# tkkiran/Robust-Conditional-GAN

Measured on AMD Instinct MI355X. Metric: images/sec G+D train step (CIFAR-10 RCGAN bs=64), higher is better.
Workload: dtype bf16

## Files before the change

include/rcgan_hip.h:

```cpp
#ifndef RCGAN_HIP_H
#define RCGAN_HIP_H

#include <stddef.h>
#include <stdint.h>

#ifdef __cplusplus
extern "C" {
#endif

#define RCGAN_OK 0
#define RCGAN_EINVALID_ARG (-1)
#define RCGAN_EUNSUPPORTED_SHAPE (-2)
#define RCGAN_EWORKSPACE_TOO_SMALL (-3)
#define RCGAN_EHIP (-4)
#define RCGAN_ERCCL (-5)

#define RCGAN_F32 0
#define RCGAN_BF16 1
#define RCGAN_F16 2

#define RCGAN_ACT_NONE 0
#define RCGAN_ACT_RELU 1
#define RCGAN_ACT_LRELU 2
#define RCGAN_ACT_TANH 3
// ... 225 lines not shown
int rcgan_conv_rf_prepare(rcgan_ctx* ctx, int n, const rcgan_conv_desc* descs, const void* const* prepared, void* const* frags);
int rcgan_fragments_prepare(rcgan_ctx* ctx, const void* const* trunk_prepared, void* trunk_frag, int n, const rcgan_conv_desc* descs,
                            const void* const* prepared, void* const* frags);
int rcgan_conv2d_rf(rcgan_ctx* ctx, const rcgan_conv_desc* d, int backward, const void* x, const void* frag, const float* bias,
                    const void* mask_x, const void* residual, void* y);

int rcgan_dblock2_ok(const rcgan_conv_desc* d, const void* conv1_frag, const void* dblock2_frag);
size_t rcgan_dblock2_fragment_bytes(void);
int rcgan_fragments_prepare_dblock2(rcgan_ctx* ctx, const void* const* trunk_prepared, void* trunk_frag, int n, const rcgan_conv_desc* descs,
                                    const void* const* prepared, void* const* frags, const void* conv2_prepared,
                                    const void* shortcut_prepared, void* dblock2_frag);
int rcgan_dblock2_fwd(rcgan_ctx* ctx, const rcgan_conv_desc* d, const void* x, const void* conv1_frag, const void* dblock2_frag,
                      const float* bias1, const float* bias2, const float* bias_shortcut, void* h, void* xp, void* y);
int rcgan_dblock2_bwd(rcgan_ctx* ctx, const rcgan_conv_desc* d, const void* dy, const void* h, const void* x, const void* conv1_frag,
                      const void* dblock2_frag, void* dh, void* dx);

int rcgan_dblock1_ok(const rcgan_conv_desc* d, const void* dblock1_frag);
size_t rcgan_dblock1_fragment_bytes(void);
int rcgan_fragments_prepare_dblocks(rcgan_ctx* ctx, const void* const* trunk_prepared, void* trunk_frag, int n, const rcgan_conv_desc* descs,
                                    const void* const* prepared, void* const* frags, const void* conv2_prepared,
                                    const void* shortcut_prepared, void* dblock2_frag, const void* block1_conv2_prepared, void* dblock1_frag);
int rcgan_dblock1_fwd(rcgan_ctx* ctx, const rcgan_conv_desc* d, const void* x, const void* conv1_prepared, const void* shortcut_prepared,
                      const void* dblock1_frag, const float* bias1, const float* bias2, const float* bias_shortcut, void* h, void* xp, void* y);
size_t rcgan_proj_head_workspace_bytes(int n, int d, int v);
typedef struct {
  int n, d, v, e_dim;
  int rows_a, kind_a, kind_b;
  float weight;
  const int32_t* labels_a; const float* wts_a; float* dwts_a;
  const int32_t* labels_b; const float* wts_b; float* dwts_b;
  const void* x; void* dx;
  int x_dtype, hw, act;
  const float* E_pre;
  void* defer_ws;
  size_t defer_ws_bytes;
} rcgan_head_desc;
int rcgan_proj_head_fwd_bwd(rcgan_ctx* ctx, const rcgan_head_desc* hd, const float* feat, const float* w_out, const float* sigma_out,
                            const float* b_out, const float* table, const float* w_e, const float* sigma_e, const float* b_e,
                            float* loss_acc, float* logits, float* dfeat, float* dw_out, float* db_out, float* dtable, float* dw_e,
                            float* db_e, void* ws, size_t ws_bytes);
int rcgan_head_flush(rcgan_ctx* ctx);

typedef struct {
  float weight;
  const float* anchor_a; const float* anchor_b;
  const float* gate;
// ... 136 lines not shown
```

robust-conditional-gan_amd/_lib.py:

```python
import ctypes as C
import os

_HERE = os.path.dirname(os.path.abspath(__file__))
LIB_PATH = os.environ.get("RCGAN_LIB_PATH") or os.path.join(_HERE, "librcgan_hip.so")
LIB_PATH_F16 = os.environ.get("RCGAN_LIB_PATH_F16") or os.path.join(_HERE, "librcgan_hip_f16.so")

F32, BF16, F16 = 0, 1, 2
ACT_NONE, ACT_RELU, ACT_LRELU, ACT_TANH, ACT_SIGMOID = 0, 1, 2, 3, 4
CONV_IN_UPSAMPLE2X, CONV_IN_RELU, CONV_ACCUMULATE, CONV_FORCE_DIRECT, CONV_OUT_MEANPOOL2, CONV_RESID_UPSAMPLE2X = 1, 2, 4, 8, 16, 32
LOSS_HINGE_REAL, LOSS_HINGE_FAKE, LOSS_NEG_MEAN, LOSS_CE_ONES, LOSS_CE_ZEROS = 0, 1, 2, 3, 4
QUERY_TR_READ = 0
AUG_COLOR, AUG_TRANSLATION, AUG_CUTOUT = 1, 2, 4
AUG_POLICIES = {"color": AUG_COLOR, "translation": AUG_TRANSLATION, "cutout": AUG_CUTOUT}
F32_PRECISION_HIGHEST, F32_PRECISION_HIGH = 0, 1
F32_PRECISIONS = {"highest": F32_PRECISION_HIGHEST, "high": F32_PRECISION_HIGH}

RCGAN_EHIP, RCGAN_ERCCL = -4, -5
EINVALID_ARG, EUNSUPPORTED_SHAPE, EWORKSPACE_TOO_SMALL = -1, -2, -3
ERRORS = {-1: "RCGAN_EINVALID_ARG", -2: "RCGAN_EUNSUPPORTED_SHAPE", -3: "RCGAN_EWORKSPACE_TOO_SMALL",
          -4: "RCGAN_EHIP", -5: "RCGAN_ERCCL"}


def source_hash():
    import glob
# ... 172 lines not shown
    "rcgan_proj_logit_fwd": (I, [P, I, I, P, P, P, P]),
    "rcgan_proj_logit_bwd": (I, [P, I, I, P, P, P, P, P, P, I]),
    "rcgan_proj_logit_all_fwd": (I, [P, I, I, I, P, P, P, P]),
    "rcgan_proj_logit_all_bwd": (I, [P, I, I, I, P, P, P, P, P, P, I]),
    "rcgan_loss_fwd_bwd": (I, [P, I, I, I, P, P, F, P, P, P]),
    "rcgan_bce_onehot_fwd_bwd": (I, [P, I, I, P, P, F, P, P]),
    "rcgan_dtrunk": (I, [P, I, I, P, P, P, P, P]),
    "rcgan_dtrunk_pooled": (I, [P, I, I, P, P, P, P, P, P, P, P]),
    "rcgan_dtrunk_prepare": (I, [P, P, P]),
    "rcgan_conv_rf_ok": (I, [C.POINTER(ConvDesc)]),
    "rcgan_conv_rf_fragment_bytes": (SZ, [C.POINTER(ConvDesc)]),
    "rcgan_conv_rf_prepare": (I, [P, I, C.POINTER(ConvDesc), P, P]),
    "rcgan_fragments_prepare": (I, [P, P, P, I, C.POINTER(ConvDesc), P, P]),
    "rcgan_conv2d_rf": (I, [P, C.POINTER(ConvDesc), I, P, P, P, P, P, P]),
    "rcgan_dblock2_ok": (I, [C.POINTER(ConvDesc), P, P]),
    "rcgan_dblock2_fragment_bytes": (SZ, []),
    "rcgan_fragments_prepare_dblock2": (I, [P, P, P, I, C.POINTER(ConvDesc), P, P, P, P, P]),
    "rcgan_dblock2_fwd": (I, [P, C.POINTER(ConvDesc), P, P, P, P, P, P, P, P, P]),
    "rcgan_dblock2_bwd": (I, [P, C.POINTER(ConvDesc), P, P, P, P, P, P, P]),
    "rcgan_dblock1_ok": (I, [C.POINTER(ConvDesc), P]),
    "rcgan_dblock1_fragment_bytes": (SZ, []),
    "rcgan_fragments_prepare_dblocks": (I, [P, P, P, I, C.POINTER(ConvDesc), P, P, P, P, P, P, P]),
    "rcgan_dblock1_fwd": (I, [P, C.POINTER(ConvDesc), P, P, P, P, P, P, P, P, P, P]),
    "rcgan_dtrunk_fragment_bytes": (SZ, []),
    "rcgan_head_flush": (I, [P]),
    "rcgan_proj_head_fwd_bwd": (I, [P, C.POINTER(HeadDesc)] + [P] * 16 + [P, SZ]),
    "rcgan_recover_mse_fwd_bwd": (I, [P, I, I, I, I, P, P, P, P, P, P, P, SZ]),
    "rcgan_softmax_rows_fwd": (I, [P, I, I, P, P]),
    "rcgan_softmax_rows_bwd": (I, [P, I, I, P, P, P, I]),
    "rcgan_softmax_xent_workspace_bytes": (SZ, [I]),
    "rcgan_softmax_xent_fwd_bwd": (I, [P, I, I, P, P, F, P, P, P, P, SZ]),
    "rcgan_softmax_xent_forward_fwd_bwd": (I, [P, I, I, P, P, P, F, P, P, P, P, P, P, SZ]),
    "rcgan_shortcut_a_fwd": (I, [P, I, I, I, I, I, P, P]),
    "rcgan_shortcut_a_bwd": (I, [P, I, I, I, I, I, P, P, I]),
    "rcgan_diffaugment_fwd": (I, [P, I, I, I, I, I, P, P, P, P]),
    "rcgan_diffaugment_bwd": (I, [P, I, I, I, I, I, P, P, P, I]),
    "rcgan_diffaugment_gated_fwd": (I, [P, I, I, I, I, I, P, P, P, P, P, P, P]),
    "rcgan_diffaugment_sampled_bwd": (I, [P, I, I, I, I, P, P, P, P, I]),
    "rcgan_ada_update": (I, [P, I, P, I, P, P, F, F, I]),
    "rcgan_loss_reg_fwd_bwd": (I, [P, I, I, I, P, P, F, P, P, P, C.POINTER(LossReg)]),
    "rcgan_proj_head_reg_fwd_bwd": (I, [P, C.POINTER(HeadDesc)] + [P] * 16 + [P, SZ, C.POINTER(LossReg)]),
    "rcgan_lecam_update": (I, [P, I, I, P, I, P, P, P, P, P, F]),
    "rcgan_pair_diversity_workspace_bytes": (SZ, [I]),
    "rcgan_pair_diversity_fwd_bwd": (I, [P, I, I, I, I, P, P, P, F, F, P, P, I, P, P, SZ]),
    "rcgan_class_moments_bytes": (SZ, [I, I]),
    "rcgan_class_moments_accum": (I, [P, I, I, I, P, P, P]),
# ... 72 lines not shown
```

robust-conditional-gan_amd/csrc/api.hip:

```cpp
#include "conv_wgrad.h"
#include "small_gemm.h"
#include "step_inputs.h"
#include "conv_image.h"
#include "gather_plan.h"


size_t direct_wgrad_ws_bytes(const rcgan_conv_desc* d);
template <typename T> int direct_fwd(rcgan_ctx*, const rcgan_conv_desc*, const T*, const float*, const float*, const float*, T*, int n_cols = 0);
template <typename T> int direct_dgrad(rcgan_ctx*, const rcgan_conv_desc*, const T*, const float*, const float*, const float*, const T*, T*, int);
template <typename T> int direct_wgrad(rcgan_ctx*, const rcgan_conv_desc*, const T*, const T*, float*, float*, int, void*, size_t);
template <typename T> int direct_wgrad_cols(rcgan_ctx*, const rcgan_conv_desc*, const T*, const T*, int, const float*, float*, int, void*, size_t);
size_t direct_wgrad_cols_ws_bytes(const rcgan_conv_desc* d, int c1);
template <typename T> int colsum_launch(rcgan_ctx*, const T*, long, int, float*, int, float*);
template <typename T> int linear_fwd(rcgan_ctx*, long, long, long, const T*, const float*, const float*, const float*, T*);
template <typename T> int linear_dgrad(rcgan_ctx*, long, long, long, const T*, const float*, const float*, T*, int);
template <typename T> int linear_wgrad(rcgan_ctx*, long, long, long, const T*, const T*, float*, float*, int, void*, size_t);
size_t linear_wgrad_ws_bytes(long m, long k, long n);
template <typename T> int sumpool2_masked_launch(rcgan_ctx*, int, int, int, int, const T*, const T*, T*, int);
int small_fwd_kind(const rcgan_conv_desc* d);
int small_dgrad_kind(const rcgan_conv_desc* d);
int small_wgrad_kind(const rcgan_conv_desc* d);
size_t small_wgrad_ws_bytes(const rcgan_conv_desc* d);
template <typename T> int small_fwd(rcgan_ctx*, const rcgan_conv_desc*, int, const T*, const float*, const float*, T*);
template <typename T> int small_dgrad(rcgan_ctx*, const rcgan_conv_desc*, int, const T*, const float*, T*, int);
// ... 732 lines not shown
    const bool scratch = up && a.phase == MFMA_FORM_PLAIN;
    if (scratch) a.out = (bf16_t*)target;
    a.mask = (relu && !scratch) ? (const bf16_t*)x : nullptr;
    a.resid = (const bf16_t*)residual;
    rc = mfma_conv_launch(ctx, a);
    if (rc || !scratch) return rc;
  } else if (mask == nullptr && !up && img_side(d)) {
    rc = img_dgrad(ctx, d, dy, prepared, target, acc_now);
    if (rc) return rc;
  } else if (int kind = (mask == nullptr && !up) ? small_dgrad_kind(d) : 0) {
    RC_DISPATCH_DTYPE(ctx, d->dtype, rc = small_dgrad<T>(ctx, d, kind, (const T*)dy, (const float*)prepared, (T*)target, acc_now));
    if (rc) return rc;
  } else {
    RC_DISPATCH_DTYPE(ctx, d->dtype, rc = direct_dgrad<T>(ctx, d, (const T*)dy, (const float*)prepared, nullptr, nullptr, (const T*)mask, (T*)target, acc_now));
    if (rc) return rc;
  }
  if (up) {
    RC_DISPATCH_DTYPE(ctx, d->dtype, rc = sumpool2_masked_launch<T>(ctx, d->n, d->h, d->w, d->cin, (const T*)ws, relu ? (const T*)x : (const T*)nullptr, (T*)dx, acc));
    if (rc) return rc;
  }
  return RCGAN_OK;
}

int rcgan_deconv2d_fwd(rcgan_ctx* ctx, const rcgan_conv_desc* d, const void* x, const float* w, const float* bias, void* y) {
  int rc = check_desc(ctx, d);
  if (rc) return rc;
  RC_DISPATCH_DTYPE(ctx, d->dtype, return direct_dgrad<T>(ctx, d, (const T*)x, w, nullptr, bias, (const T*)nullptr, (T*)y, 0));
  return RCGAN_OK;
}

int rcgan_deconv2d_bwd_data(rcgan_ctx* ctx, const rcgan_conv_desc* d, const void* dy, const float* w, void* dx) {
  return rcgan_deconv2d_bwd_data_cols(ctx, d, dy, w, dx, 0);
}

int rcgan_deconv2d_bwd_data_cols(rcgan_ctx* ctx, const rcgan_conv_desc* d, const void* dy, const float* w, void* dx, int n_cols) {
  int rc = check_desc(ctx, d);
  if (rc) return rc;
  RC_REQUIRE(ctx, n_cols >= 0 && n_cols <= d->cout, "n_cols %d of %d input channels", n_cols, d->cout);
  RC_DISPATCH_DTYPE(ctx, d->dtype, return direct_fwd<T>(ctx, d, (const T*)dy, w, nullptr, nullptr, (T*)dx, n_cols));
  return RCGAN_OK;
}

int rcgan_deconv2d_bwd_weight(rcgan_ctx* ctx, const rcgan_conv_desc* d, const void* x, const void* dy, float* dw, float* dbias,
                              int accumulate, void* ws, size_t ws_bytes) {
  int rc = check_desc(ctx, d);
  if (rc) return rc;
// ... 134 lines not shown
```

robust-conditional-gan_amd/csrc/conv_mfma.h:

```cpp
#pragma once
#include "common.h"

struct ImgWArgs;

struct MfmaConvArgs {
  const bf16_t* in;
  const bf16_t* wt;
  const float* bias;
  const bf16_t* mask;
  const bf16_t* resid;
  int resid_up;
  bf16_t* out;
  const bf16_t* zero;
  int N, H, W, Cin, Cout, KH, KW, PT, PL;
  int up, relu_in, accumulate;
  int cm;
  int lw, lh;
  long M;
  unsigned long long* stamps;
  const bf16_t* wph;
  int phase;
  float* stats;
  const float* bn_mean = nullptr;
  const float* bn_rstd = nullptr;
// ... 33 lines not shown
int direct_prepare_launch(rcgan_ctx* ctx, const float* w, const float* sigma, float* out, long total);
int mfma_selftest(rcgan_ctx* ctx, int* host_result);
extern int g_use_tr;
int ensure_selftest(rcgan_ctx* ctx);
int check_desc(rcgan_ctx* ctx, const rcgan_conv_desc* d);
int img_side(const rcgan_conv_desc* d);
size_t img_extra_offset(const rcgan_conv_desc* d);
size_t img_extra_bytes(const rcgan_conv_desc* d);
size_t img_wgrad_ws_bytes(const rcgan_conv_desc* d);
int img_prepare_launch(rcgan_ctx* ctx, const rcgan_conv_desc* d, const float* w, const float* sigma, void* prepared);
int img_fwd(rcgan_ctx* ctx, const rcgan_conv_desc* d, const void* x, const void* prepared, const float* bias, void* y);
int img_dgrad(rcgan_ctx* ctx, const rcgan_conv_desc* d, const void* dy, const void* prepared, void* dx, int accumulate);
bool img_fwd_bn_ok(const rcgan_conv_desc* d);
int img_fwd_bn(rcgan_ctx* ctx, const rcgan_conv_desc* d, const void* x, const void* prepared, const float* bias, void* y,
               const float* mean, const float* rstd, const float* gamma, const float* beta, const int32_t* labels, int segments, int act);
int img_wgrad_plan(rcgan_ctx* ctx, const rcgan_conv_desc* d, const void* x, const void* dy, int target_wgs, ImgWArgs* a, int* cb, int* nwg);
int img_wgrad(rcgan_ctx* ctx, const rcgan_conv_desc* d, const void* x, const void* dy, float* dw, float* dbias, int accumulate,
              void* ws, size_t ws_bytes);
int mfma_conv8_launch(rcgan_ctx* ctx, const MfmaConvArgs& a, bool wide, bool halo_patch);
bool mfma_conv8_halo_takes(const MfmaConvArgs& a);
int mfma_conv8_halo_launch(rcgan_ctx* ctx, const MfmaConvArgs& a);
bool mfma_conv8n_halo_takes(const MfmaConvArgs& a);
int mfma_conv8n_halo_launch(rcgan_ctx* ctx, const MfmaConvArgs& a);
int mfma_conv_bn_route(const MfmaConvArgs& a);
struct SmallGemmArgs;
struct StepInputsArgs;
int conv_prepare_batch_launch(rcgan_ctx* ctx, const rcgan_prepare_item* items, int n, const SmallGemmArgs* gemm = nullptr,
                              const StepInputsArgs* inputs = nullptr, const rcgan_frag_item* frags = nullptr, int n_frags = 0);
```

robust-conditional-gan_amd/csrc/conv_mfma.hip:

```cpp
#include <vector>
#include "conv_mfma.h"
#include "small_gemm.h"
#include "step_inputs.h"
#include "mfma_util.h"

#define LDS_PITCH 72

template <int BM, int BN>
__global__ __launch_bounds__(256) void conv_mfma_kernel(MfmaConvArgs a) {
  extern __shared__ __attribute__((aligned(16))) unsigned char smem[];
  bf16_t* As = (bf16_t*)smem;
  bf16_t* Bs = As + 2 * BM * LDS_PITCH;
  constexpr int AR = BM / 32, BR = BN / 32;
  constexpr int TM = BM / 2, TN = BN / 2;
  constexpr int NI = TN / 16, NJ = TM / 16;

  const int tid = threadIdx.x, lane = tid & 63, wave = tid >> 6;
  const int wm = wave & 1, wn = wave >> 1;
  const long m0 = (long)blockIdx.x * BM;
  const int co0 = blockIdx.y * BN;
  const int chunk = tid & 7, lrow = tid >> 3;
  const int K = a.KH * a.KW * a.Cin;
  const int KT = K / 64;
  const int Hs = a.up ? (a.H >> 1) : a.H, Ws = a.up ? (a.W >> 1) : a.W;
// ... 963 lines not shown
  const bool off32 = (long)a.N * a.H * a.W * a.Cin < (1L << 32);
  const long b8 = (long)cdiv(a.M, 256) * (a.Cout / 256), b8n = (long)cdiv(a.M, 256) * (a.Cout / 128);
  const bool fit8 = 4 * b8 >= 3 * (long)cdiv(b8, 256) * 256;
  if (a.Cout % 256 == 0 && a.zero != nullptr && off32 && b8 >= p8_min && fit8) return (halo && !a.stats && mfma_conv8_halo_takes(b)) ? CR_H8 : CR_P8;
  if (a.Cout % 128 == 0 && a.zero != nullptr && b8n >= p8n_min) return (halo_n && mfma_conv8n_halo_takes(b)) ? CR_H8N : CR_P8N;
  if (a.Cout % 256 == 0 && b8 >= t256_min && a.zero != nullptr) return CR_T256;
  if (a.Cout % 128 == 0 && b8n >= t256_min && a.zero != nullptr) return CR_T256N;
  if (a.Cout % 128 == 0 && (long)cdiv(a.M, 128) * (a.Cout / 128) >= t128_min) return CR_T128;
  return CR_64;
}

bool mfma_conv_is_p8(const MfmaConvArgs& a) {
  if (a.phase != MFMA_FORM_PLAIN || a.Cin % 64 || a.Cout % 64) return false;
  const ConvRoute r = mfma_conv_route(a);
  return r == CR_H8 || r == CR_P8;
}

int mfma_conv_bn_route(const MfmaConvArgs& a) {
  if (a.phase != MFMA_FORM_PLAIN || a.Cin % 64 || a.Cout % 64 || a.zero == nullptr || a.stats || a.relu_in || a.Cin > 1024) return 0;
  const ConvRoute r = mfma_conv_route(a);
  return r == CR_H8 ? 1 : r == CR_H8N ? 2 : 0;
}

int mfma_conv_launch(rcgan_ctx* ctx, const MfmaConvArgs& a_in) {
  MfmaConvArgs a = a_in;
  a.stamps = (unsigned long long*)ctx->dbg_stamps;
  if (a.Cin % 64 || a.Cout % 64) RC_FAIL(ctx, RCGAN_EUNSUPPORTED_SHAPE, "channels %d -> %d", a.Cin, a.Cout);
  const ConvRoute r = mfma_conv_route(a);
  if (a.bn_mean && !(a.phase == MFMA_FORM_PLAIN && !a.stats && !a.relu_in && a.Cin <= 1024 && a.zero != nullptr && (r == CR_H8 || r == CR_H8N)))
    RC_FAIL(ctx, RCGAN_EUNSUPPORTED_SHAPE, "batch norm on the staged input needs a halo-patch kernel (rcgan_conv_bn_in_ok)");
  if (a.stats && !(a.phase == MFMA_FORM_PLAIN && a.zero != nullptr && (r == CR_H8 || r == CR_P8)))
    RC_FAIL(ctx, RCGAN_EUNSUPPORTED_SHAPE, "tile statistics need the 256 x 256 kernel (rcgan_conv_stats_ok)");
  switch (r) {
    case CR_H8: case CR_P8: return mfma_conv8_launch(ctx, a, true, r == CR_H8);
    case CR_H8N: case CR_P8N: return mfma_conv8_launch(ctx, a, false, r == CR_H8N);
    case CR_PHASE_KS2: return a.phase == MFMA_FORM_PHASE ? launch_conv_glds_phase<64, 64, 2, 2, 1>(ctx, a) : launch_conv_glds_phase<64, 64, 2, 2, 2>(ctx, a);
    case CR_PHASE: return a.phase == MFMA_FORM_PHASE ? launch_conv_glds_phase<64, 64, 2, 1, 1>(ctx, a) : launch_conv_glds_phase<64, 64, 2, 1, 2>(ctx, a);
    case CR_T256: return launch_conv_glds<256, 256, 2>(ctx, a);
    case CR_T256N: return launch_conv_glds<256, 128, 2>(ctx, a);
    case CR_T128: return launch_conv_mfma<128, 128>(ctx, a);
    default: return launch_conv_mfma<64, 64>(ctx, a);
  }
}

int mfma_prepare_launch(rcgan_ctx* ctx, const float* w, const float* sigma, bf16_t* wt, bf16_t* wd, int T, int Cin, int Cout) {
  long total = (long)T * Cin * Cout;
// ... 58 lines not shown
```

robust-conditional-gan_amd/csrc/conv_mfma8h.hip:

```cpp
#include "conv_mfma.h"
#include "mfma_util.h"

#ifndef H8_ABLATE
#define H8_ABLATE 0
#endif

namespace {

template <int N> __device__ __forceinline__ void wait_vm() {
  if constexpr (N == 0) asm volatile("s_waitcnt vmcnt(0)" ::: "memory");
  else if constexpr (N == 1) asm volatile("s_waitcnt vmcnt(1)" ::: "memory");
  else if constexpr (N == 2) asm volatile("s_waitcnt vmcnt(2)" ::: "memory");
  else if constexpr (N == 3) asm volatile("s_waitcnt vmcnt(3)" ::: "memory");
  else if constexpr (N == 4) asm volatile("s_waitcnt vmcnt(4)" ::: "memory");
  else if constexpr (N == 5) asm volatile("s_waitcnt vmcnt(5)" ::: "memory");
  else if constexpr (N == 6) asm volatile("s_waitcnt vmcnt(6)" ::: "memory");
  else if constexpr (N == 7) asm volatile("s_waitcnt vmcnt(7)" ::: "memory");
  else if constexpr (N == 8) asm volatile("s_waitcnt vmcnt(8)" ::: "memory");
  else if constexpr (N == 9) asm volatile("s_waitcnt vmcnt(9)" ::: "memory");
  else if constexpr (N == 10) asm volatile("s_waitcnt vmcnt(10)" ::: "memory");
  else if constexpr (N == 11) asm volatile("s_waitcnt vmcnt(11)" ::: "memory");
  else if constexpr (N == 12) asm volatile("s_waitcnt vmcnt(12)" ::: "memory");
  else static_assert(N == 0, "unsupported vmcnt immediate");
}
// ... 690 lines not shown
  if (a.phase == 1) return a.up && a.wph != nullptr && (a.lw == 5 || a.lw == 6) && a.lh >= 1 && ((a.H >> 1) << (a.lw - 1)) % 256 == 0 && (a.M >> 2) % 256 == 0;
  return false;
}

template <int LW, bool RELU, bool PHM, bool BNIN = false, int NPASS = 1, bool GATHER = false>
static int launch8hn(rcgan_ctx* ctx, const MfmaConvArgs& a) {
  static bool attr_set = false;
  const size_t lds = h8n_lds_bytes(LW) + (BNIN ? 2 * H8_BN_MAX_CIN * sizeof(float) : 0);
  if (!attr_set) {
    RC_HIP(ctx, hipFuncSetAttribute((const void*)conv_mfma_h8n_kernel<LW, RELU, PHM, BNIN, NPASS, GATHER>, hipFuncAttributeMaxDynamicSharedMemorySize, (int)lds));
    attr_set = true;
  }
  dim3 grid(cdiv(a.M, 256 * NPASS), a.Cout / 128);
  {
    ProfScope ps(ctx, RCGAN_PROF_CONV_P8N, 2.0 * (double)a.M * (GATHER ? 36 : 9) * a.Cin * a.Cout,
                 2.0 * (double)a.M * (GATHER ? 16 : PHM ? 4 : 9) * a.Cin * a.Cout);
    if (BNIN && ps.on) ctx->prof_bn_in++;
    hipLaunchKernelGGL((conv_mfma_h8n_kernel<LW, RELU, PHM, BNIN, NPASS, GATHER>), grid, dim3(512), lds, ctx->stream, a);
  }
  RC_LAUNCH_CHECK(ctx);
  return RCGAN_OK;
}

int mfma_conv8n_halo_launch(rcgan_ctx* ctx, const MfmaConvArgs& a) {
  if (a.bn_mean) {
    if (a.relu_in || a.Cin > H8_BN_MAX_CIN || (a.bn_act != RCGAN_ACT_NONE && a.bn_act != RCGAN_ACT_RELU))
      RC_FAIL(ctx, RCGAN_EUNSUPPORTED_SHAPE, "batch norm on the staged patch: no input ReLU, Cin <= %d, activation none / ReLU", H8_BN_MAX_CIN);
    if (a.phase == 1) return a.lw == 6 ? launch8hn<5, false, true, true>(ctx, a) : launch8hn<4, false, true, true>(ctx, a);
    return a.lw == 5 ? launch8hn<5, false, false, true>(ctx, a) : launch8hn<4, false, false, true>(ctx, a);
  }
  if (a.phase == 2) {
    if (a.lw == 6) return a.relu_in ? launch8hn<5, true, false, false, 1, true>(ctx, a) : launch8hn<5, false, false, false, 1, true>(ctx, a);
    return a.relu_in ? launch8hn<4, true, false, false, 1, true>(ctx, a) : launch8hn<4, false, false, false, 1, true>(ctx, a);
  }
  if (a.phase == 1) {
    static int two = -1;
    if (two < 0) { const char* e = getenv("RCGAN_H8N_TWO_PASS"); two = e ? atoi(e) : 1; }
    if (two && a.Cin <= 128 && (a.M / 512) * (a.Cout / 128) >= 190) {
      if (a.lw == 6) return a.relu_in ? launch8hn<5, true, true, false, 2>(ctx, a) : launch8hn<5, false, true, false, 2>(ctx, a);
      return a.relu_in ? launch8hn<4, true, true, false, 2>(ctx, a) : launch8hn<4, false, true, false, 2>(ctx, a);
    }
    if (a.lw == 6) return a.relu_in ? launch8hn<5, true, true>(ctx, a) : launch8hn<5, false, true>(ctx, a);
    return a.relu_in ? launch8hn<4, true, true>(ctx, a) : launch8hn<4, false, true>(ctx, a);
  }
  if (a.lw == 5) return a.relu_in ? launch8hn<5, true, false>(ctx, a) : launch8hn<5, false, false>(ctx, a);
  return a.relu_in ? launch8hn<4, true, false>(ctx, a) : launch8hn<4, false, false>(ctx, a);
}
```

robust-conditional-gan_amd/csrc/conv_rf.hip:

```cpp
#include <type_traits>

#include "conv_mfma.h"
#include "mfma_util.h"
#include "rf_asm.h"

namespace {

struct RfArgs {
  const bf16_t* in;
  const bf16_t* wfrag;
  const float* bias;
  const bf16_t* mask;
  const bf16_t* resid;
  bf16_t* out;
  const bf16_t* zero;
  int accumulate, relu_in;
  int H, W, lbpi, Cout;
  int res_lw, res_lh;
  long M;
  unsigned long long* stamps;
};

constexpr int RF_ROWS = 8;
constexpr int RF_UPFRONT = 4;
// ... 238 lines not shown
                                    const void* const* prepared, void* const* frags, const void* conv2_prepared,
                                    const void* shortcut_prepared, void* dblock2_frag, const void* block1_conv2_prepared, void* dblock1_frag) {
  if (!ctx) return RCGAN_EINVALID_ARG;
  RC_REQUIRE(ctx, (block1_conv2_prepared != nullptr) == (dblock1_frag != nullptr), "the input block's copy needs its prepared filter and a destination");
  RC_REQUIRE(ctx, n >= 0 && n <= 12 && (n == 0 || (descs && prepared && frags)) && (!trunk_prepared || trunk_frag), "bad arguments");
  RC_REQUIRE(ctx, (conv2_prepared != nullptr) == (dblock2_frag != nullptr) && (shortcut_prepared != nullptr) == (dblock2_frag != nullptr),
             "the down block's copies need both prepared filters and a destination");
  RC_REQUIRE(ctx, (dblock2_frag ? DB2_FRAG_ITEMS : 0) + (dblock1_frag ? DB1_FRAG_ITEMS : 0) + (trunk_prepared ? 16 : 0) + 2 * n <=
                      (int)(sizeof(FragBatch::it) / sizeof(FragItem)),
             "more fragment items than one launch holds");
  FragBatch b;
  int m = 0, maxchunks = 0;
  if (dblock2_frag) {
    const rcgan_conv_desc d2 = {1, 16, 16, 128, 128, 3, 3, 1, RCGAN_H16, RCGAN_CONV_OUT_MEANPOOL2};
    const rcgan_conv_desc ds = {1, 8, 8, 128, 128, 1, 1, 1, RCGAN_H16, 0};
    dblock2_frag_items((const bf16_t*)conv2_prepared + mfma_prepared_sum_fwd(&d2), (const bf16_t*)shortcut_prepared,
                       (const bf16_t*)conv2_prepared + mfma_prepared_sum_bwd(&d2), (const bf16_t*)shortcut_prepared + mfma_prepared_rot(&ds),
                       (bf16_t*)dblock2_frag, b.it);
    m = DB2_FRAG_ITEMS;
    maxchunks = b.it[0].chunks;
  }
  if (dblock1_frag) {
    const rcgan_conv_desc d2 = {1, 32, 32, 128, 128, 3, 3, 1, RCGAN_H16, RCGAN_CONV_OUT_MEANPOOL2};
    dblock1_frag_items((const bf16_t*)block1_conv2_prepared + mfma_prepared_sum_fwd(&d2), (bf16_t*)dblock1_frag, b.it + m);
    if (b.it[m].chunks > maxchunks) maxchunks = b.it[m].chunks;
    m += DB1_FRAG_ITEMS;
  }
  if (trunk_prepared) {
    const long elems = 9L * 128 * 128;
    for (int i = 0; i < 8; ++i) {
      RC_REQUIRE(ctx, trunk_prepared[i], "stage layer %d: null pointer", i);
      b.it[m++] = FragItem{(const bf16_t*)trunk_prepared[i], (bf16_t*)trunk_frag + i * elems, 1152, 2, 36, 1, (int)(elems / 8)};
      b.it[m++] = FragItem{(const bf16_t*)trunk_prepared[7 - i] + elems, (bf16_t*)trunk_frag + (8 + i) * elems, 1152, 2, 36, 1, (int)(elems / 8)};
    }
    if ((int)(elems / 8) > maxchunks) maxchunks = (int)(elems / 8);
  }
  for (int i = 0; i < n; ++i) {
    const rcgan_conv_desc* d = descs + i;
    RC_REQUIRE(ctx, rf_takes(d) && prepared[i] && frags[i], "filter %d: not a register-filter shape / null pointer", i);
    const long elems = 9L * d->cin * d->cout;
    for (int dir = 0; dir < 2; ++dir) {
      const int kc = dir ? d->cout : d->cin;
      b.it[m++] = FragItem{(const bf16_t*)prepared[i] + dir * elems, (bf16_t*)frags[i] + dir * elems, 9 * kc, 4, 18, kc / 64, (int)(elems / 8)};
    }
    if ((int)(elems / 8) > maxchunks) maxchunks = (int)(elems / 8);
  }
  if (m == 0) return RCGAN_OK;
// ... 33 lines not shown
```

robust-conditional-gan_amd/csrc/rf_asm.h:

```cpp
#pragma once
#include <type_traits>

#include "mfma_util.h"

typedef __attribute__((ext_vector_type(4))) int i32x4_t;

#if RCGAN_HALF_FP16
#define RF_MFMA "v_mfma_f32_16x16x32_f16"
#else
#define RF_MFMA "v_mfma_f32_16x16x32_bf16"
#endif

template <int OFF> __device__ __forceinline__ void rf_load_a(i32x4_t& dst, const void* p) {
  asm volatile("global_load_dwordx4 %0, %1, off offset:%2" : "=a"(dst) : "v"(p), "n"(OFF) : "memory");
}
template <int OFF> __device__ __forceinline__ void rf_load_v(i32x4_t& dst, const void* p) {
  asm volatile("global_load_dwordx4 %0, %1, off offset:%2" : "=v"(dst) : "v"(p), "n"(OFF) : "memory");
}
template <int OFF> __device__ __forceinline__ void rf_load_a_inplace(i32x4_t& dst, const void* p) {
  asm volatile("global_load_dwordx4 %0, %1, off offset:%2" : "+a"(dst) : "v"(p), "n"(OFF) : "memory");
}
__device__ __forceinline__ void rf_mfma_a(f32x4_t& acc, const i32x4_t& w, const bf16x8_t& x) {
  asm volatile(RF_MFMA " %0, %1, %2, %0" : "+v"(acc) : "a"(w), "v"(x) : "memory");
}
// ... 15 lines not shown
template <int N> __device__ __forceinline__ void rf_wait() { asm volatile("s_waitcnt vmcnt(%0)" :: "n"(N) : "memory"); }
__device__ __forceinline__ void rf_barrier() { asm volatile("s_waitcnt lgkmcnt(0)\n\ts_barrier" ::: "memory"); }

template <int I, int N, typename F> __device__ __forceinline__ void rf_for(F&& f) {
  if constexpr (I < N) { f(std::integral_constant<int, I>{}); rf_for<I + 1, N>(f); }
}

struct FragItem { const bf16_t* src; bf16_t* dst; int K, ctn, ss, nsl, chunks; };

constexpr long DB2_FRAG_CONV2 = 16L * 128 * 128;
constexpr long DB2_FRAG_SHORT = 128L * 128;
constexpr long DB2_FRAG_CONV2_BWD = DB2_FRAG_CONV2 + DB2_FRAG_SHORT;
constexpr long DB2_FRAG_SHORT_BWD = DB2_FRAG_CONV2_BWD + DB2_FRAG_CONV2;
constexpr long DB2_FRAG_ELEMS = DB2_FRAG_SHORT_BWD + DB2_FRAG_SHORT;
constexpr int DB2_FRAG_ITEMS = 4;
inline void dblock2_frag_items(const bf16_t* conv2_sum_fwd, const bf16_t* shortcut_fwd, const bf16_t* conv2_sum_bwd, const bf16_t* shortcut_rot,
                               bf16_t* frag, FragItem* it) {
  it[0] = FragItem{conv2_sum_fwd, frag, 2048, 2, 64, 1, (int)(DB2_FRAG_CONV2 / 8)};
  it[1] = FragItem{shortcut_fwd, frag + DB2_FRAG_CONV2, 128, 2, 4, 1, (int)(DB2_FRAG_SHORT / 8)};
  it[2] = FragItem{conv2_sum_bwd, frag + DB2_FRAG_CONV2_BWD, 512, 2, 16, 1, (int)(DB2_FRAG_CONV2 / 8)};
  it[3] = FragItem{shortcut_rot, frag + DB2_FRAG_SHORT_BWD, 128, 2, 4, 1, (int)(DB2_FRAG_SHORT / 8)};
}

constexpr long DB1_FRAG_ELEMS = 16L * 128 * 128;
constexpr int DB1_FRAG_ITEMS = 1;
inline void dblock1_frag_items(const bf16_t* conv2_sum_fwd, bf16_t* frag, FragItem* it) {
  it[0] = FragItem{conv2_sum_fwd, frag, 2048, 2, 64, 1, (int)(DB1_FRAG_ELEMS / 8)};
}
```

robust-conditional-gan_amd/ops.py:

```python
import ctypes as C
import os

import torch

from . import _lib as L
from .runtime import DT


def _p(t):
    return C.c_void_p(t.ptr) if t is not None else None


def same_pad(n, k, s):
    out = -(-n // s)
    tot = max((out - 1) * s + k - n, 0)
    return out, tot // 2


def zeros_like_grad(ctx, t):
    g = ctx.empty(t.shape, t.dtype)
    ctx.check(ctx.lib.rcgan_fill_f32(ctx.h, (g.nbytes + 3) // 4, g.ptr, 0.0))
    return g


# ... 483 lines not shown
            dh, dx = d_block2_bwd(ctx, d, dy, h, x, w1, frag)
            for wr, (desc, operand, w, b), g in zip(wreq, layers, (dy, dh, dy)):
                if wr:
                    ctx.defer_wgrad(desc, operand, g, w.grad_target(), b.grad if b.req else None)
            h.grad = dh
            x.grad = dx
        ctx.record(bw)
    return out


FUSED_DBLOCK2_BWD = os.environ.get("RCGAN_FUSED_DBLOCK2_BWD", "1") != "0"

FUSED_DBLOCK1 = os.environ.get("RCGAN_FUSED_DBLOCK1", "1") != "0"


def d_block1_ok(ctx, x, frag):
    if not FUSED_DBLOCK1 or frag is None or len(x.shape) != 4 or x.dtype == L.F32:
        return False
    n, h, w, c = x.shape
    d = L.ConvDesc(n, h, w, c, 128, 3, 3, 1, x.dtype, 0)
    return bool(ctx.lib.rcgan_dblock1_ok(C.byref(d), _p(frag)))


def d_block1(ctx, x, ws, bs, w1, b1, w2, b2, frag, pooled=None, _saved=None):
    n = x.shape[0]
    d = L.ConvDesc(n, 32, 32, 3, 128, 3, 3, 1, x.dtype, 0)
    ds = L.ConvDesc(n, 16, 16, 3, 128, 1, 1, 1, x.dtype, 0)
    h = ctx.empty((n, 32, 32, 128), x.dtype)
    y = ctx.empty((n, 16, 16, 128), x.dtype)
    xp = ctx.empty((n, 16, 16, 3), x.dtype) if pooled is None else None
    ctx.check(ctx.lib.rcgan_dblock1_fwd(ctx.h, C.byref(d), _p(x), _p(w1.prepared(d)), _p(ws.prepared(ds)), _p(frag), _p(b1), _p(b2), _p(bs),
                                        _p(h), _p(xp), _p(y)))
    xp = pooled if pooled is not None else meanpool2(ctx, x, _done=xp)
    t = conv2d(ctx, xp, ws, bs, 1, _done=y)
    h = conv2d(ctx, x, w1, b1, 3, _done=h)
    if _saved is not None:
        _saved += [h, xp]
    return conv2d_meanpool(ctx, h, w2, b2, in_relu=True, accumulate_into=t, _done=True)


def d_trunk_ok(ctx, x):
    return x.dtype != L.F32 and tuple(x.shape[1:]) == (8, 8, 128)


def d_trunk(ctx, x, blocks, pool=None, frag=None):
    n = x.shape[0]
    assert d_trunk_ok(ctx, x) and len(blocks) == 4 and pool in (None, L.ACT_RELU)
    desc = L.ConvDesc(n, 8, 8, 128, 128, 3, 3, 1, x.dtype, L.CONV_IN_RELU)
    arr = lambda ts: (C.c_void_p * 8)(*[(t.ptr if t is not None else None) for t in ts])
    flat = []
    for w1, b1, w2, b2 in blocks:
        flat += [(w1, b1), (w2, b2)]
    preps = [w.prepared(desc) for w, _ in flat]
    outs = [ctx.empty(x.shape, x.dtype) for _ in range(8)]
    if frag is None:
        frag = DT(ctx.arena.alloc(ctx.lib.rcgan_dtrunk_fragment_bytes()), (ctx.lib.rcgan_dtrunk_fragment_bytes(),), "u8", ctx.arena.buf)
        ctx.check(ctx.lib.rcgan_dtrunk_prepare(ctx.h, arr(preps), _p(frag)))
    feat = ctx.empty((n, 128), L.F32) if pool is not None else None
    ctx.check(ctx.lib.rcgan_dtrunk_pooled(ctx.h, n, 0, _p(x), _p(frag), arr([b for _, b in flat]), None, arr(outs), _p(feat), None, None))
    y = outs[7]
    y.pooled, y.pool_grad = ((feat, pool) if feat is not None else None), None
# ... 767 lines not shown
```

Baseline: 62940.

## Add fused backward kernel for discriminator input block conv2 dgrad with ReLU mask

```diff
diff --git a/include/rcgan_hip.h b/include/rcgan_hip.h
--- a/include/rcgan_hip.h
+++ b/include/rcgan_hip.h
@@ -271,6 +271,8 @@
                                     const void* shortcut_prepared, void* dblock2_frag, const void* block1_conv2_prepared, void* dblock1_frag);
 int rcgan_dblock1_fwd(rcgan_ctx* ctx, const rcgan_conv_desc* d, const void* x, const void* conv1_prepared, const void* shortcut_prepared,
                       const void* dblock1_frag, const float* bias1, const float* bias2, const float* bias_shortcut, void* h, void* xp, void* y);
+int rcgan_dblock1_bwd_same_bits(const rcgan_conv_desc* d);
+int rcgan_dblock1_bwd(rcgan_ctx* ctx, const rcgan_conv_desc* d, const void* dy, const void* h, const void* dblock1_frag, void* dh, void* dx);
 size_t rcgan_proj_head_workspace_bytes(int n, int d, int v);
 typedef struct {
   int n, d, v, e_dim;
diff --git a/robust-conditional-gan_amd/_lib.py b/robust-conditional-gan_amd/_lib.py
--- a/robust-conditional-gan_amd/_lib.py
+++ b/robust-conditional-gan_amd/_lib.py
@@ -218,6 +218,8 @@
     "rcgan_dblock1_fragment_bytes": (SZ, []),
     "rcgan_fragments_prepare_dblocks": (I, [P, P, P, I, C.POINTER(ConvDesc), P, P, P, P, P, P, P]),
     "rcgan_dblock1_fwd": (I, [P, C.POINTER(ConvDesc), P, P, P, P, P, P, P, P, P, P]),
+    "rcgan_dblock1_bwd_same_bits": (I, [C.POINTER(ConvDesc)]),
+    "rcgan_dblock1_bwd": (I, [P, C.POINTER(ConvDesc), P, P, P, P, P]),
     "rcgan_dtrunk_fragment_bytes": (SZ, []),
     "rcgan_head_flush": (I, [P]),
     "rcgan_proj_head_fwd_bwd": (I, [P, C.POINTER(HeadDesc)] + [P] * 16 + [P, SZ]),
diff --git a/robust-conditional-gan_amd/csrc/api.hip b/robust-conditional-gan_amd/csrc/api.hip
--- a/robust-conditional-gan_amd/csrc/api.hip
+++ b/robust-conditional-gan_amd/csrc/api.hip
@@ -778,6 +778,14 @@
   return RCGAN_OK;
 }
 
+int rcgan_dblock1_bwd_same_bits(const rcgan_conv_desc* d) {
+  if (!d || d->dtype != RCGAN_H16 || d->n < 1) return 0;
+  const rcgan_conv_desc d2 = {d->n, 32, 32, 128, 128, 3, 3, 1, d->dtype, RCGAN_CONV_OUT_MEANPOOL2 | RCGAN_CONV_IN_RELU};
+  MfmaConvArgs a;
+  if (mfma_conv_pose(nullptr, &d2, CONV_DGRAD, nullptr, nullptr, nullptr, false, nullptr, &a)) return 0;
+  return mfma_conv_is_h8n_two_pass(a) ? 1 : 0;
+}
+
 int rcgan_deconv2d_fwd(rcgan_ctx* ctx, const rcgan_conv_desc* d, const void* x, const float* w, const float* bias, void* y) {
   int rc = check_desc(ctx, d);
   if (rc) return rc;
diff --git a/robust-conditional-gan_amd/csrc/conv_dblock1_bwd.hip b/robust-conditional-gan_amd/csrc/conv_dblock1_bwd.hip
--- /dev/null
+++ b/robust-conditional-gan_amd/csrc/conv_dblock1_bwd.hip
@@ -0,0 +1,233 @@
+#include <type_traits>
+
+#include "conv_mfma.h"
+#include "mfma_util.h"
+#include "rf_asm.h"
+
+namespace {
+
+constexpr int B1_YW = 18;
+constexpr int B1_YNPP = 10 * B1_YW;
+constexpr int B1_YDMA = B1_YNPP * 16 / 64;
+constexpr int B1_YPW = (B1_YDMA + 3) / 4;
+constexpr int B1_YBYTES = B1_YDMA * 1024;
+constexpr int B1_NT = 8;
+constexpr int B1_CLS = B1_NT * 16 * 256;
+constexpr int B1_GDEP = B1_CLS / 1024 / 4;
+constexpr int B1_LDS = B1_YBYTES + 2 * B1_CLS;
+constexpr int B1_RING = 32;
+constexpr int B1_FIRST = 8;
+constexpr int B1_STEPS = 64;
+constexpr int B1_GROUPS = B1_STEPS / 16;
+static_assert(B1_YNPP * 16 % 64 == 0, "the dy patch is whole deposits");
+static_assert(B1_STEPS % B1_RING == 0 && B1_RING * 8 == 256, "the ring is the 256 AccVGPRs");
+static_assert(B1_LDS <= 160 * 1024, "LDS of one CU");
+
+struct Db1BwdArgs {
+  const bf16_t *dy, *h;
+  const bf16_t* w2;
+  bf16_t* dh;
+  const bf16_t* zero;
+  unsigned long long* stamps;
+};
+
+constexpr int b1_upto(int v) {
+  const int fill = B1_FIRST + 1 + 2 * v, lap = v + B1_RING;
+  const int s = fill < lap ? fill : lap;
+  return s < B1_STEPS - 1 ? s : B1_STEPS - 1;
+}
+constexpr int b1_gbase(int g) { return g < 2 ? B1_GDEP * g : 16 * (g - 1); }
+constexpr int b1_deposit_group(int v, int k) {
+  int seen = 0;
+  for (int g = 0; g < B1_GROUPS; ++g)
+    if (v >= b1_gbase(g) && v < b1_gbase(g) + B1_GDEP) { if (seen == k) return g; ++seen; }
+  return -1;
+}
+constexpr int b1_loads_in(int v) {
+  int c = 2 * (b1_upto(v) - b1_upto(v - 1));
+  for (int k = 0; k < 2; ++k) c += b1_deposit_group(v, k) >= 0 ? 1 : 0;
+  return c;
+}
+constexpr int b1_cap(int c) { return c > 63 ? 63 : c; }
+constexpr int b1_behind(int u) {
+  int c = 0, from = 0;
+  if (u < B1_FIRST) c = 2 * (B1_FIRST - 1 - u);
+  else {
+    for (int v = 0; v < u; ++v)
+      if (b1_upto(v - 1) < u && u <= b1_upto(v)) {
+        c = 2 * (b1_upto(v) - u);
+        for (int k = 0; k < 2; ++k) c += b1_deposit_group(v, k) >= 0 ? 1 : 0;
+        from = v + 1;
+      }
+  }
+  for (int v = from; v < u; ++v) c += b1_loads_in(v);
+  return b1_cap(c);
+}
+constexpr int b1_behind_mask(int g) {
+  const int last = b1_gbase(g) + B1_GDEP - 1;
+  int c = 0;
+  for (int k = 0; k < 2; ++k) c += b1_deposit_group(last, k) > g ? 1 : 0;
+  for (int v = last + 1; v <= 16 * g + 15; ++v) c += b1_loads_in(v);
+  return b1_cap(c);
+}
+static_assert(b1_upto(-1) == B1_FIRST - 1 && b1_upto(B1_STEPS - 1) == B1_STEPS - 1, "every K-step is requested once");
+static_assert(b1_gbase(B1_GROUPS - 1) + B1_GDEP - 1 < 16 * (B1_GROUPS - 1) + 15 && b1_gbase(1) + B1_GDEP - 1 <= 15 && B1_GDEP <= 16,
+              "a class's deposits are out before its epilogue");
+
+__global__ __launch_bounds__(256) void conv_dblock1_bwd_kernel(Db1BwdArgs a) {
+  extern __shared__ __attribute__((aligned(16))) unsigned char smem[];
+  const int tid = threadIdx.x, lane = tid & 63;
+  const int wave = __builtin_amdgcn_readfirstlane(tid >> 6);
+  const int r = lane & 15, kc = lane >> 4;
+  const int n = (int)blockIdx.x >> 1, hb = (int)blockIdx.x & 1;
+  unsigned char* const dyp = smem;
+  unsigned char* const hmask = smem + B1_YBYTES;
+  auto stamp = [&](int k) __attribute__((always_inline)) {
+    if (a.stamps && tid == 0) a.stamps[(long)blockIdx.x * 16 + k] = __builtin_amdgcn_s_memtime();
+  };
+  stamp(0);
+
+  const unsigned lds0 = (unsigned)(size_t)(__attribute__((address_space(3))) unsigned char*)smem;
+  {
+    const bf16_t* const img = a.dy + (long)n * 256 * 128;
+#pragma unroll
+    for (int i = 0; i < B1_YPW; ++i) {
+      const int q = i * 4 + wave;
+      if (q < B1_YDMA) {
+        const int c = q * 64 + lane, pp = c >> 4, sp = c & 15;
+        const int pr = pp / B1_YW, pc = pp - pr * B1_YW;
+        const int ih = 8 * hb - 1 + pr, iw = pc - 1;
+        const bool ok = ih >= 0 && ih < 16 && iw >= 0 && iw < 16;
+        const int off = ((ih * 16 + iw) * 128 + ((sp ^ (pp & 15)) << 3)) * 2;
+        const char* src = ok ? (const char*)img + off : (const char*)a.zero;
+        glds16_asm(src, lds0 + q * 1024);
+      }
+    }
+  }
+  i32x4_t WA[B1_RING / 2][4];
+  const bf16_t* const w2l = a.w2 + (long)wave * (16 * 1024) + lane * 8;
+  auto wsrc = [&](auto ic) __attribute__((always_inline)) -> const bf16_t* {
+    constexpr int u = decltype(ic)::value, q = (u >> 4) & 3, s = u & 15, c = s >> 3, tap = (s >> 1) & 3, ks = s & 1;
+    return w2l + q * (64 * 1024) + (tap * 4 + 2 * c + ks) * 1024;
+  };
+  auto ring_load = [&](auto ic) __attribute__((always_inline)) {
+    constexpr int u = decltype(ic)::value, slot = u % B1_RING;
+    const bf16_t* const p = wsrc(ic);
+    if constexpr (u < B1_RING) {
+      rf_load_a<0>(WA[slot >> 1][2 * (slot & 1)], p); rf_load_a<1024>(WA[slot >> 1][2 * (slot & 1) + 1], p);
+    } else {
+      rf_load_a_inplace<0>(WA[slot >> 1][2 * (slot & 1)], p); rf_load_a_inplace<1024>(WA[slot >> 1][2 * (slot & 1) + 1], p);
+    }
+  };
+  rf_for<0, B1_FIRST>(ring_load);
+  const bf16_t* const himg = a.h + ((long)n * 32 + 16 * hb) * 32 * 128;
+  auto mask_load = [&](int g, int i) __attribute__((always_inline)) {
+    const int ph = g >> 1, pw = g & 1;
+    const int j = i * 4 + wave;
+    int ln;
+    asm volatile("v_mov_b32 %0, %1" : "=v"(ln) : "v"(lane));
+    const int pi = j * 4 + (ln >> 4), sp = ln & 15;
+    const int hp = (2 * (pi >> 4) + ph) * 32 + 2 * (pi & 15) + pw;
+    glds16_asm((const char*)himg + (hp * 128 + ((sp ^ (pi & 15)) << 3)) * 2, lds0 + B1_YBYTES + (g & 1) * B1_CLS + j * 1024);
+  };
+  stamp(1);
+  rf_wait<2 * B1_FIRST>();
+  rf_barrier();
+  stamp(2);
+
+  int rr = r;
+  asm volatile("" : "+v"(rr));
+  auto xread = [&](auto ic, bf16x8_t (&xf)[B1_NT]) __attribute__((always_inline)) {
+    constexpr int u = decltype(ic)::value, q = u >> 4, s = u & 15, c = s >> 3, tap = (s >> 1) & 3, ks = s & 1;
+    constexpr int ph = q >> 1, pw = q & 1, ta = tap >> 1, tb = tap & 1, cq = 2 * c + ks;
+#pragma unroll
+    for (int pt = 0; pt < B1_NT; ++pt) {
+      const int pp = (pt + ta + ph) * B1_YW + tb + pw + rr;
+      xf[pt] = *(const bf16x8_t*)(dyp + pp * 256 + (((cq * 4 + kc) ^ (pp & 15)) << 4));
+    }
+  };
+  f32x4_t acc1[B1_NT][2];
+  bf16x8_t xf1[2][B1_NT];
+  xread(std::integral_constant<int, 0>{}, xf1[0]);
+  rf_for<0, B1_STEPS>([&](auto ic) __attribute__((always_inline)) {
+    constexpr int u = decltype(ic)::value, slot = u % B1_RING, g = u >> 4, s = u & 15, ph = g >> 1, pw = g & 1;
+    if constexpr (s == 15) asm volatile("" : "+v"(rr));
+    if constexpr (u + 1 < B1_STEPS) xread(std::integral_constant<int, u + 1>{}, xf1[(u + 1) & 1]);
+    rf_wait<b1_behind(u)>();
+#pragma unroll
+    for (int ct = 0; ct < 2; ++ct)
+#pragma unroll
+      for (int pt = 0; pt < B1_NT; ++pt) {
+        const i32x4_t& w = WA[slot >> 1][2 * (slot & 1) + ct];
+        if constexpr (s == 0) rf_mfma_a0(acc1[pt][ct], w, xf1[u & 1][pt]);
+        else rf_mfma_a(acc1[pt][ct], w, xf1[u & 1][pt]);
+      }
+    rf_for<b1_upto(u - 1) + 1, b1_upto(u) + 1>(ring_load);
+    if constexpr (b1_deposit_group(u, 0) >= 0) mask_load(b1_deposit_group(u, 0), u - b1_gbase(b1_deposit_group(u, 0)));
+    if constexpr (b1_deposit_group(u, 1) >= 0) mask_load(b1_deposit_group(u, 1), u - b1_gbase(b1_deposit_group(u, 1)));
+    if constexpr (s == 15) {
+      rf_wait<b1_behind_mask(g)>();
+      rf_barrier();
+      asm volatile("s_nop 15\n\ts_nop 15" ::: "memory");
+      int ln;
+      asm volatile("v_mov_b32 %0, %1" : "=v"(ln) : "v"(lane));
+      const int r = ln & 15, c8 = wave * 32 + ((ln >> 4) & 1) * 16 + (ln >> 5) * 8;
+#pragma unroll
+      for (int pt = 0; pt < B1_NT; ++pt) {
+        float x[4], y[4];
+#pragma unroll
+        for (int k = 0; k < 4; ++k) {
+          x[k] = acc1[pt][0][k] + 0.f;
+          y[k] = acc1[pt][1][k] + 0.f;
+          swap16(x[k], y[k]);
+        }
+        const int pi = pt * 16 + r;
+        const uint4 m = *(const uint4*)(hmask + (g & 1) * B1_CLS + pi * 256 + (((c8 >> 3) ^ r) << 4));
+        const uint32_t mw[4] = {m.x, m.y, m.z, m.w};
+#pragma unroll
+        for (int k = 0; k < 2; ++k) {
+          if (!(h16_lo(mw[k]) > 0.f)) x[2 * k] = 0.f;
+          if (!(h16_hi(mw[k]) > 0.f)) x[2 * k + 1] = 0.f;
+          if (!(h16_lo(mw[2 + k]) > 0.f)) y[2 * k] = 0.f;
+          if (!(h16_hi(mw[2 + k]) > 0.f)) y[2 * k + 1] = 0.f;
+        }
+        const uint4 pk = make_uint4(pack_h16x2(x[0], x[1]), pack_h16x2(x[2], x[3]), pack_h16x2(y[0], y[1]), pack_h16x2(y[2], y[3]));
+        const int hp = (2 * pt + ph) * 32 + 2 * r + pw;
+        *(uint4*)(a.dh + (((long)n * 32 + 16 * hb) * 32 + hp) * 128 + c8) = pk;
+      }
+      stamp(3 + g);
+      if constexpr (g + 2 < B1_GROUPS) rf_barrier();
+    }
+  });
+  if (a.stamps) {
+    asm volatile("s_waitcnt vmcnt(0)" ::: "memory");
+    stamp(7);
+  }
+}
+
+}
+
+extern "C" {
+
+int rcgan_dblock1_bwd(rcgan_ctx* ctx, const rcgan_conv_desc* d, const void* dy, const void* h, const void* dblock1_frag, void* dh, void* dx) {
+  if (!ctx) return RCGAN_EINVALID_ARG;
+  RC_REQUIRE(ctx, rcgan_dblock1_ok(d, dblock1_frag), "not the 32x32x3 input block / missing fragment copy (rcgan_dblock1_ok)");
+  RC_REQUIRE(ctx, dy && h && (dh || dx), "null argument");
+  if (dx) RC_FAIL(ctx, RCGAN_EUNSUPPORTED_SHAPE, "the images' gradient is not part of this launch: dx must be null");
+  Db1BwdArgs a;
+  a.dy = (const bf16_t*)dy; a.h = (const bf16_t*)h;
+  a.w2 = (const bf16_t*)dblock1_frag + DB1_FRAG_CONV2_BWD;
+  a.dh = (bf16_t*)dh;
+  a.zero = (const bf16_t*)ctx->zero_page;
+  a.stamps = (unsigned long long*)ctx->dbg_stamps;
+  static bool attr_set = false;
+  if (!attr_set) {
+    RC_HIP(ctx, hipFuncSetAttribute((const void*)conv_dblock1_bwd_kernel, hipFuncAttributeMaxDynamicSharedMemorySize, (int)B1_LDS));
+    attr_set = true;
+  }
+  hipLaunchKernelGGL(conv_dblock1_bwd_kernel, dim3(2 * d->n), dim3(256), B1_LDS, ctx->stream, a);
+  RC_LAUNCH_CHECK(ctx);
+  return RCGAN_OK;
+}
+
+}
diff --git a/robust-conditional-gan_amd/csrc/conv_mfma.h b/robust-conditional-gan_amd/csrc/conv_mfma.h
--- a/robust-conditional-gan_amd/csrc/conv_mfma.h
+++ b/robust-conditional-gan_amd/csrc/conv_mfma.h
@@ -79,6 +79,8 @@
 int mfma_conv8_halo_launch(rcgan_ctx* ctx, const MfmaConvArgs& a);
 bool mfma_conv8n_halo_takes(const MfmaConvArgs& a);
 int mfma_conv8n_halo_launch(rcgan_ctx* ctx, const MfmaConvArgs& a);
+bool mfma_conv8n_two_pass(const MfmaConvArgs& a);
+bool mfma_conv_is_h8n_two_pass(const MfmaConvArgs& a);
 int mfma_conv_bn_route(const MfmaConvArgs& a);
 struct SmallGemmArgs;
 struct StepInputsArgs;
diff --git a/robust-conditional-gan_amd/csrc/conv_mfma.hip b/robust-conditional-gan_amd/csrc/conv_mfma.hip
--- a/robust-conditional-gan_amd/csrc/conv_mfma.hip
+++ b/robust-conditional-gan_amd/csrc/conv_mfma.hip
@@ -1009,6 +1009,11 @@
   return r == CR_H8 ? 1 : r == CR_H8N ? 2 : 0;
 }
 
+bool mfma_conv_is_h8n_two_pass(const MfmaConvArgs& a) {
+  if (a.phase != MFMA_FORM_PHASE || a.Cin % 64 || a.Cout % 64 || a.bn_mean || a.stats) return false;
+  return mfma_conv_route(a) == CR_H8N && mfma_conv8n_two_pass(a);
+}
+
 int mfma_conv_launch(rcgan_ctx* ctx, const MfmaConvArgs& a_in) {
   MfmaConvArgs a = a_in;
   a.stamps = (unsigned long long*)ctx->dbg_stamps;
diff --git a/robust-conditional-gan_amd/csrc/conv_mfma8h.hip b/robust-conditional-gan_amd/csrc/conv_mfma8h.hip
--- a/robust-conditional-gan_amd/csrc/conv_mfma8h.hip
+++ b/robust-conditional-gan_amd/csrc/conv_mfma8h.hip
@@ -736,6 +736,12 @@
   return RCGAN_OK;
 }
 
+bool mfma_conv8n_two_pass(const MfmaConvArgs& a) {
+  static int two = -1;
+  if (two < 0) { const char* e = getenv("RCGAN_H8N_TWO_PASS"); two = e ? atoi(e) : 1; }
+  return a.phase == 1 && !a.bn_mean && two && a.Cin <= 128 && (a.M / 512) * (a.Cout / 128) >= 190;
+}
+
 int mfma_conv8n_halo_launch(rcgan_ctx* ctx, const MfmaConvArgs& a) {
   if (a.bn_mean) {
     if (a.relu_in || a.Cin > H8_BN_MAX_CIN || (a.bn_act != RCGAN_ACT_NONE && a.bn_act != RCGAN_ACT_RELU))
@@ -748,9 +754,7 @@
     return a.relu_in ? launch8hn<4, true, false, false, 1, true>(ctx, a) : launch8hn<4, false, false, false, 1, true>(ctx, a);
   }
   if (a.phase == 1) {
-    static int two = -1;
-    if (two < 0) { const char* e = getenv("RCGAN_H8N_TWO_PASS"); two = e ? atoi(e) : 1; }
-    if (two && a.Cin <= 128 && (a.M / 512) * (a.Cout / 128) >= 190) {
+    if (mfma_conv8n_two_pass(a)) {
       if (a.lw == 6) return a.relu_in ? launch8hn<5, true, true, false, 2>(ctx, a) : launch8hn<5, false, true, false, 2>(ctx, a);
       return a.relu_in ? launch8hn<4, true, true, false, 2>(ctx, a) : launch8hn<4, false, true, false, 2>(ctx, a);
     }
diff --git a/robust-conditional-gan_amd/csrc/conv_rf.hip b/robust-conditional-gan_amd/csrc/conv_rf.hip
--- a/robust-conditional-gan_amd/csrc/conv_rf.hip
+++ b/robust-conditional-gan_amd/csrc/conv_rf.hip
@@ -284,7 +284,8 @@
   }
   if (dblock1_frag) {
     const rcgan_conv_desc d2 = {1, 32, 32, 128, 128, 3, 3, 1, RCGAN_H16, RCGAN_CONV_OUT_MEANPOOL2};
-    dblock1_frag_items((const bf16_t*)block1_conv2_prepared + mfma_prepared_sum_fwd(&d2), (bf16_t*)dblock1_frag, b.it + m);
+    dblock1_frag_items((const bf16_t*)block1_conv2_prepared + mfma_prepared_sum_fwd(&d2),
+                       (const bf16_t*)block1_conv2_prepared + mfma_prepared_sum_bwd(&d2), (bf16_t*)dblock1_frag, b.it + m);
     if (b.it[m].chunks > maxchunks) maxchunks = b.it[m].chunks;
     m += DB1_FRAG_ITEMS;
   }
diff --git a/robust-conditional-gan_amd/csrc/rf_asm.h b/robust-conditional-gan_amd/csrc/rf_asm.h
--- a/robust-conditional-gan_amd/csrc/rf_asm.h
+++ b/robust-conditional-gan_amd/csrc/rf_asm.h
@@ -61,8 +61,11 @@
   it[3] = FragItem{shortcut_rot, frag + DB2_FRAG_SHORT_BWD, 128, 2, 4, 1, (int)(DB2_FRAG_SHORT / 8)};
 }
 
-constexpr long DB1_FRAG_ELEMS = 16L * 128 * 128;
-constexpr int DB1_FRAG_ITEMS = 1;
-inline void dblock1_frag_items(const bf16_t* conv2_sum_fwd, bf16_t* frag, FragItem* it) {
-  it[0] = FragItem{conv2_sum_fwd, frag, 2048, 2, 64, 1, (int)(DB1_FRAG_ELEMS / 8)};
+constexpr long DB1_FRAG_CONV2 = 16L * 128 * 128;
+constexpr long DB1_FRAG_CONV2_BWD = DB1_FRAG_CONV2;
+constexpr long DB1_FRAG_ELEMS = DB1_FRAG_CONV2_BWD + DB1_FRAG_CONV2;
+constexpr int DB1_FRAG_ITEMS = 2;
+inline void dblock1_frag_items(const bf16_t* conv2_sum_fwd, const bf16_t* conv2_sum_bwd, bf16_t* frag, FragItem* it) {
+  it[0] = FragItem{conv2_sum_fwd, frag, 2048, 2, 64, 1, (int)(DB1_FRAG_CONV2 / 8)};
+  it[1] = FragItem{conv2_sum_bwd, frag + DB1_FRAG_CONV2_BWD, 512, 2, 16, 1, (int)(DB1_FRAG_CONV2 / 8)};
 }
diff --git a/robust-conditional-gan_amd/ops.py b/robust-conditional-gan_amd/ops.py
--- a/robust-conditional-gan_amd/ops.py
+++ b/robust-conditional-gan_amd/ops.py
@@ -529,6 +529,12 @@
     return bool(ctx.lib.rcgan_dblock1_ok(C.byref(d), _p(frag)))
 
 
+def d_block1_bwd(ctx, d, dy, h, frag):
+    dh = ctx.empty(h.shape, h.dtype)
+    ctx.check(ctx.lib.rcgan_dblock1_bwd(ctx.h, C.byref(d), _p(dy), _p(h), _p(frag), _p(dh), None))
+    return dh
+
+
 def d_block1(ctx, x, ws, bs, w1, b1, w2, b2, frag, pooled=None, _saved=None):
     n = x.shape[0]
     d = L.ConvDesc(n, 32, 32, 3, 128, 3, 3, 1, x.dtype, 0)
@@ -538,12 +544,42 @@
     xp = ctx.empty((n, 16, 16, 3), x.dtype) if pooled is None else None
     ctx.check(ctx.lib.rcgan_dblock1_fwd(ctx.h, C.byref(d), _p(x), _p(w1.prepared(d)), _p(ws.prepared(ds)), _p(frag), _p(b1), _p(b2), _p(bs),
                                         _p(h), _p(xp), _p(y)))
+    mark = len(ctx.tape)
     xp = pooled if pooled is not None else meanpool2(ctx, x, _done=xp)
     t = conv2d(ctx, xp, ws, bs, 1, _done=y)
     h = conv2d(ctx, x, w1, b1, 3, _done=h)
     if _saved is not None:
         _saved += [h, xp]
-    return conv2d_meanpool(ctx, h, w2, b2, in_relu=True, accumulate_into=t, _done=True)
+    out = conv2d_meanpool(ctx, h, w2, b2, in_relu=True, accumulate_into=t, _done=True)
+    entries = ctx.tape[mark:]
+    if FUSED_DBLOCK1_BWD and len(entries) >= 3:
+        del ctx.tape[mark:]
+        d2 = L.ConvDesc(n, 32, 32, 128, 128, 3, 3, 1, x.dtype, L.CONV_OUT_MEANPOOL2 | L.CONV_IN_RELU)
+        layers = ((d2, h, w2, b2), (d, x, w1, b1), (ds, xp, ws, bs))
+        wreq = [w.req for _, _, w, _ in layers]
+
+        def bw():
+            dy = out.grad
+            if dy is None:
+                return
+            fused = (not x.req and not xp.req and h.req and ctx.group_wgrads and h.grad is None
+                     and all(wr or not b.req for wr, (_, _, _, b) in zip(wreq, layers))
+                     and (not wreq[0] or ctx.lib.rcgan_conv_wgrad_pool_ok(C.byref(d2)))
+                     and bool(ctx.lib.rcgan_dblock1_bwd_same_bits(C.byref(d))))
+            if not fused:
+                for fn in reversed(entries):
+                    fn()
+                return
+            dh = d_block1_bwd(ctx, d, dy, h, frag)
+            for wr, (desc, operand, w, b), g in zip(wreq, layers, (dy, dh, dy)):
+                if wr:
+                    ctx.defer_wgrad(desc, operand, g, w.grad_target(), b.grad if b.req else None)
+            h.grad = dh
+        ctx.record(bw)
+    return out
+
+
+FUSED_DBLOCK1_BWD = os.environ.get("RCGAN_FUSED_DBLOCK1_BWD", "1") != "0"
 
 
 def d_trunk_ok(ctx, x):
```

After: 63140, median of 3. No clear change (+0.3%).
